# gtonkinhill/tracs

Hardware: AMD Instinct MI355X
Metric: sample-pairs/sec for 10kx5Mbp SNP+transcluster distance (higher is better)
Workload: dtype u32; 1 GPU; 10000 samples x 5000000 sites, consensus (ACGTN) alignment, mu = 0.0001 per sample + 0.01 N (SURVEY 8d): pairsnp (d + compared sites) + transcluster (P, E(K)), all 49995000 pairs; samples=10000, sites=5000000, pairs=49995000, encoding=consensus, kernel=mfma, distinct_keys=174015, partition=one rank: no exchange, workload_name=sparse, streams=1, checksum_d=49010657734

## Files before the change

tracs_amd/csrc/site_lists.hip:

```cpp
#include "pairsnp_kernels.h"

#include <algorithm>
#include <cstdio>
#include <cstddef>
#include <cstdlib>

namespace tracs {

struct SiteLists {
    uint4 *lines = nullptr;
    unsigned long long n_lines = 0;
    unsigned long long *p_off = nullptr;
    unsigned *p_ent = nullptr;
    uint4 *qlines = nullptr;
    unsigned long long n_qlines = 0;
    unsigned qw = 32;
    unsigned long long *s_off = nullptr;
    unsigned *s_ent = nullptr;
    unsigned *c_p = nullptr;
    uint4 *T = nullptr;
    size_t tgroups = 0;
    unsigned short *slots = nullptr;
    size_t batches = 0;
    uint4 *nnl_mask = nullptr;
    uint4 *lst_mask = nullptr;
    unsigned *off_lst = nullptr;
    size_t sites = 0, groups = 0;
    unsigned long long tot_p = 0, tot_nnl = 0;
    unsigned max_row = 0;
    unsigned max_row_pad = 0;
    unsigned long long slot_lines = 0;
    unsigned rows[4] = {0, 0, 0, 0};
    int n_rows = 0;
    unsigned *ns = nullptr;
    size_t ns_words = 0;
    unsigned *site_of = nullptr;
};
constexpr int ENT_SHIFT = 5;
constexpr unsigned ENT_HOLE = 0xFFFFFFFFu;
constexpr unsigned ENT_LONG = 0x80000000u;

__device__ __forceinline__ unsigned word_of(const uint4 &v, int w) { return w == 0 ? v.x : w == 1 ? v.y : w == 2 ? v.z : v.w; }

__device__ __forceinline__ unsigned lst_rank(const uint4 &m, unsigned off_g, int w, int b)
{
    unsigned r = off_g;
    if (w > 0) r += __popc(m.x);
    if (w > 1) r += __popc(m.y);
    if (w > 2) r += __popc(m.z);
    return r + __popc(word_of(m, w) & ((1u << b) - 1u));
}

__device__ __forceinline__ bool row_wanted(const MinorBuild &mb, size_t s)
{
    if (mb.n_rows == 0) return true;
    return (s >= mb.rows[0] && s < mb.rows[1]) || (mb.n_rows > 1 && s >= mb.rows[2] && s < mb.rows[3]);
}

#ifndef TRACS_PL_THREADS
#define TRACS_PL_THREADS 512
#endif
constexpr unsigned PL_THREADS = TRACS_PL_THREADS, PL_MIN = 1024, PL_CAP = 8192, PL_CHUNK = 4096, PL_PER_THREAD = PL_CHUNK / PL_THREADS;
static_assert(PL_PER_THREAD * PL_THREADS == PL_CHUNK && PL_PER_THREAD <= 32 && 64 % PL_PER_THREAD == 0, "p_lists_kernel: a thread's samples sit in one flag word");
__device__ __forceinline__ bool p_lists_in_lds(unsigned group_entries) { return group_entries >= PL_MIN && group_entries <= PL_CAP; }
constexpr unsigned SITE_THREADS = 128;

struct N8Encoder {
    uint4 *lines;
    unsigned line, next_ovf, fill, prev;
    unsigned left;
    unsigned a0, a1, a2, a3;
    static constexpr unsigned DONE = 0xFFFFu;
    __device__ __forceinline__ void put(unsigned b, bool more)
    {
        a0 = __builtin_amdgcn_alignbit(a1, a0, 8); a1 = __builtin_amdgcn_alignbit(a2, a1, 8); a2 = __builtin_amdgcn_alignbit(a3, a2, 8);
        a3 = (a3 >> 8) | (b << 24);
        fill++;
        const bool full = fill == N8_PAYLOAD;
        if ((fill & 15u) == 0u || full) {
            const unsigned nx = more ? next_ovf : N8_NONE;
            lines[(size_t)line * 8 + (full ? 7u : (fill >> 4) - 1u)] = full ? make_uint4(a1, a2, a3, nx) : make_uint4(a0, a1, a2, a3);
            if (full) {
                if (more) { line = next_ovf++; fill = 0; }
                else fill = DONE;
            }
        }
    }
    __device__ __forceinline__ void finish()
    {
        if (fill == DONE) return;
        const uint4 ones = make_uint4(0xFFFFFFFFu, 0xFFFFFFFFu, 0xFFFFFFFFu, 0xFFFFFFFFu);
        while ((fill & 15u) != 0u && fill != DONE) put(0xFFu, false);
        if (fill == DONE) return;
        for (unsigned q = fill >> 4; q < 8u; q++) lines[(size_t)line * 8 + q] = ones;
    }
};

#ifndef TRACS_SITE_WAVES
#define TRACS_SITE_WAVES 8
#endif
#if TRACS_SITE_WAVES > 0
#define TRACS_SITE_ATTR __attribute__((amdgpu_waves_per_eu(TRACS_SITE_WAVES, TRACS_SITE_WAVES)))
#else
#define TRACS_SITE_ATTR
#endif
template <unsigned PIECE_SAMPLES>
__global__ __launch_bounds__(SITE_THREADS) TRACS_SITE_ATTR void site_lists_kernel(const MinorBuild mb, size_t n_pad, unsigned n,
                                                         unsigned long long *__restrict__ p_off, unsigned *__restrict__ p_ent,
                                                         unsigned *__restrict__ qd, uint2 *__restrict__ E, unsigned *__restrict__ e_cnt,
                                                         uint4 *__restrict__ lines,
                                                         unsigned *__restrict__ c_p)
{
    constexpr unsigned PIECE_WORDS = PIECE_SAMPLES / 32, BM_STRIDE = PIECE_WORDS + 1;
    __shared__ unsigned bm[SITES_PER_GROUP * BM_STRIDE];
    __shared__ unsigned kp[SITES_PER_GROUP], ovf[SITES_PER_GROUP], curP[SITES_PER_GROUP], rk[SITES_PER_GROUP];
    __shared__ unsigned qb[SITES_PER_GROUP];
    unsigned *const curQ = ovf;
    __shared__ unsigned long long bP[SITES_PER_GROUP];
    __shared__ unsigned short queue[PIECE_SAMPLES];
    __shared__ unsigned qn[2];
    const size_t g = blockIdx.x;
    const int tid = threadIdx.x;
    const unsigned lane = tid & 63u, wave = tid >> 6;
    if (g == 0 && tid == 0) p_off[mb.sites] = mb.tot_p;
    const uint4 m4 = mb.lst_mask[g], q4 = mb.minor_mask[g];
    if ((m4.x | m4.y | m4.z | m4.w) == 0u) return;
    const unsigned m[4] = {m4.x, m4.y, m4.z, m4.w};
    const unsigned mp[4] = {q4.x, q4.y, q4.z, q4.w};
    const bool any_minor = (q4.x | q4.y | q4.z | q4.w) != 0u;
    const bool from_planes = any_minor && !p_lists_in_lds(mb.gP[g]);
    if (from_planes && tid == 0) e_cnt[g] = 0xFFFFFFFFu;
    static_assert(SITE_THREADS == SITES_PER_GROUP, "thread = site");
    const int tw = tid >> 5, tb = tid & 31;
    const bool mine = (m[tw] >> tb) & 1u;
    const bool want_n = mb.gram == 0;
    const unsigned my_cn = (mine && want_n) ? mb.cntN[g * SITES_PER_GROUP + tid] : 0u;
    {
        const unsigned c = my_cn;
        kp[tid] = (mine && ((mp[tw] >> tb) & 1u)) ? mb.cntP[g * SITES_PER_GROUP + tid] : 0u;
        ovf[tid] = mine ? n8_lines_max(c, n) - 1u : 0u;
        curP[tid] = 0;
        if (tid < 2) qn[tid] = 0;
    }
    __syncthreads();
    const Transpose32 transpose(lane);
    N8Encoder enc{lines, 0u, 0u, 0u, 0xFFFFFFFFu, 0u, 0u, 0u, 0u, 0u};
    if (mine) {
        unsigned long long pp = 0;
        unsigned po = 0, pq = 0;
        for (int t = 0; t < tid; t++) { pp += kp[t]; po += ovf[t]; pq += kp[t] / 31u; }
        const unsigned rank = lst_rank(m4, mb.off_lst[g], tw, tb);
        bP[tid] = mb.baseP[g] + pp; rk[tid] = rank;
        qb[tid] = (unsigned)(mb.sites + mb.baseQ[g] + pq);
        p_off[rank] = bP[tid];
        enc.line = rank;
        enc.left = my_cn;
        enc.next_ovf = (unsigned)(mb.sites + mb.baseO[g] + po);
    }
    __syncthreads();
    curQ[tid] = 0;
    const uint4 RX = mb.ref_x[g], RY = mb.ref_y[g];
    const uint4 *base = mb.planes + (g * NPLANES) * n_pad;
    const uint4 zero4 = make_uint4(0u, 0u, 0u, 0u);
    auto place = [&](unsigned s, unsigned st, unsigned code) {
        const unsigned slot = (code & 16u) ? atomicAdd(&curP[st], 1u) : kp[st] - 1u - atomicAdd(&curQ[st], 1u);
        const unsigned long long pos = bP[st] + slot;
        const bool is_long = kp[st] > P_SHORT_MAX;
        if (is_long) {
            const unsigned qs = slot + 1u, qt = qs / (mb.qw - 1u);
            qd[(size_t)(qt ? qb[st] + qt - 1u : rk[st]) * mb.qw + (qs - qt * (mb.qw - 1u))] = (s << ENT_SHIFT) | code;
        } else {
            p_ent[pos] = (s << ENT_SHIFT) | code;
        }
        E[pos] = (code & 16u) ? make_uint2(s, (is_long ? ENT_LONG : 0u) | (rk[st] << ENT_SHIFT) | code) : make_uint2(ENT_HOLE, 0u);
    };
    for (unsigned piece = 0; piece < n; piece += PIECE_SAMPLES) {
        const unsigned par = (piece / PIECE_SAMPLES) & 1u;
        unsigned sl = wave;
        uint4 N_next = zero4;
        unsigned long long fl_next = 0ull;
        {
            const unsigned s = piece + sl * 64u + lane;
            if (s < n) { if (want_n) N_next = base[4 * n_pad + s]; if (from_planes) fl_next = mb.flags[g * mb.flag_words + (s >> 6)]; }
        }
        for (; sl < PIECE_SAMPLES / 64u; sl += SITE_THREADS / 64u) {
            const unsigned s = piece + sl * 64u + lane;
            const uint4 N = N_next;
            const unsigned long long fl = fl_next;
            {
                const unsigned sn = s + SITE_THREADS;
                N_next = zero4; fl_next = 0ull;
                if (sl + SITE_THREADS / 64u < PIECE_SAMPLES / 64u && sn < n) { if (want_n) N_next = base[4 * n_pad + sn]; if (from_planes) fl_next = mb.flags[g * mb.flag_words + (sn >> 6)]; }
            }
            if (!want_n) {
            } else if (piece + sl * 64u < n) {
                const unsigned col = sl * 2u + (lane >> 5), r = lane & 31u;
                bm[(0u + r) * BM_STRIDE + col] = transpose(N.x & m[0]);
                bm[(32u + r) * BM_STRIDE + col] = transpose(N.y & m[1]);
                bm[(64u + r) * BM_STRIDE + col] = transpose(N.z & m[2]);
                bm[(96u + r) * BM_STRIDE + col] = transpose(N.w & m[3]);
            } else {
                const unsigned col = sl * 2u + (lane >> 5), r = lane & 31u;
                bm[(0u + r) * BM_STRIDE + col] = 0u; bm[(32u + r) * BM_STRIDE + col] = 0u;
                bm[(64u + r) * BM_STRIDE + col] = 0u; bm[(96u + r) * BM_STRIDE + col] = 0u;
            }
            const bool flagged = s < n && ((fl >> (s & 63u)) & 1ull);
            const unsigned long long fm = __ballot(flagged);
            if (fm) {
                unsigned qb = 0;
                if (lane == 0) qb = atomicAdd(&qn[par], (unsigned)__popcll(fm));
                qb = __shfl(qb, 0, 64);
                if (flagged) queue[qb + __builtin_amdgcn_mbcnt_hi((unsigned)(fm >> 32), __builtin_amdgcn_mbcnt_lo((unsigned)fm, 0u))] = (unsigned short)(s - piece);
            }
        }
        __syncthreads();
        const unsigned qcount = qn[par];
        if (tid == 0) qn[par ^ 1u] = 0;
        for (unsigned k = tid; k < qcount; k += SITE_THREADS) {
            const unsigned s = piece + queue[k];
            const uint4 A = base[s], C = base[n_pad + s], G = base[2 * n_pad + s], T = base[3 * n_pad + s];
            unsigned listed_w = 0;
#pragma unroll
            for (int w = 0; w < 4; w++) {
                const unsigned a = word_of(A, w), c = word_of(C, w), gg = word_of(G, w), t = word_of(T, w), isn = a & c & gg & t;
                const unsigned rx = word_of(RX, w), ry = word_of(RY, w);
                const unsigned ra = ~rx & ~ry, rc = rx & ~ry, rg = ~rx & ry, rt = rx & ry;
                const unsigned has_ref = (a & ra) | (c & rc) | (gg & rg) | (t & rt);
                const unsigned only_ref = ~((a ^ ra) | (c ^ rc) | (gg ^ rg) | (t ^ rt));
                unsigned pm = (a | c | gg | t) & ~isn & ~only_ref & mp[w];
                while (pm) {
                    const int b = __ffs(pm) - 1;
                    pm &= pm - 1;
                    const unsigned mask = ((a >> b) & 1u) | (((c >> b) & 1u) << 1) | (((gg >> b) & 1u) << 2) | (((t >> b) & 1u) << 3);
                    const unsigned code = (((has_ref >> b) & 1u) ? 0u : 16u) | mask;
                    place(s, (unsigned)(w * 32 + b), code);
                    listed_w += code >> 4;
                }
            }
            if (listed_w) atomicAdd(&c_p[s], listed_w);
        }
        if (mine && my_cn != 0u) {
            static_assert(PIECE_WORDS <= 64, "one bit per word of the piece");
            const unsigned *rowp = bm + (unsigned)tid * BM_STRIDE;
            unsigned long long nz = 0;
#pragma unroll
            for (unsigned c = 0; c < PIECE_WORDS; c++) nz |= (unsigned long long)(rowp[c] != 0u ? 1u : 0u) << c;
            unsigned w = 0, c = 0, gap = 0;
            bool have = false;
            for (;;) {
                if (!have) {
                    if (w == 0u) {
                        if (nz == 0ull) break;
                        c = __ffsll((long long)nz) - 1; nz &= nz - 1;
                        w = rowp[c];
                    }
                    const unsigned b = __ffs(w) - 1;
                    w &= w - 1;
                    const unsigned smp = piece + 32u * c + b;
                    gap = smp - enc.prev;
                    enc.prev = smp; enc.left--;
                    have = true;
                }
                const bool skip = gap >= N8_SKIP;
                enc.put(skip ? N8_SKIP : gap, skip || enc.left != 0u);
                if (skip) gap -= N8_SKIP; else have = false;
            }
        }
        __syncthreads();
    }
    if (mine) {
        if (want_n) enc.finish();
        if (from_planes && kp[tid] > P_SHORT_MAX) { qd[(size_t)rk[tid] * mb.qw] = kp[tid] | (curP[tid] << 16); qd[(size_t)rk[tid] * mb.qw + mb.qw - 1u] = qb[tid]; }
    }
}

__global__ __launch_bounds__(PL_THREADS) void p_lists_kernel(const MinorBuild mb, size_t n_pad, unsigned n, unsigned *__restrict__ p_ent,
                                                             unsigned *__restrict__ qd, uint2 *__restrict__ E, unsigned *__restrict__ e_cnt,
                                                             int holes, unsigned *__restrict__ c_p)
{
    __shared__ unsigned sorted[PL_CAP];
    __shared__ unsigned w1off[SITES_PER_GROUP];
    __shared__ unsigned char site_of[PL_CAP];
    __shared__ unsigned kp[SITES_PER_GROUP], loff[SITES_PER_GROUP], curP[SITES_PER_GROUP], curQ[SITES_PER_GROUP], rk[SITES_PER_GROUP], qb[SITES_PER_GROUP];
    __shared__ unsigned short queue[PL_CHUNK];
    __shared__ unsigned wtot[PL_THREADS / 64];
    const size_t g = blockIdx.x;
    const unsigned tid = threadIdx.x, lane = tid & 63u, wave = tid >> 6;
    const uint4 q4 = mb.minor_mask[g];
    if ((q4.x | q4.y | q4.z | q4.w) == 0u) return;
    const unsigned long long baseP = mb.baseP[g];
    if (!p_lists_in_lds(mb.gP[g])) return;
    if (tid < SITES_PER_GROUP) {
        const bool mine = (word_of(q4, (int)(tid >> 5)) >> (tid & 31u)) & 1u;
        kp[tid] = mine ? mb.cntP[g * SITES_PER_GROUP + tid] : 0u;
        curP[tid] = 0; curQ[tid] = 0;
    }
    __syncthreads();
    if (tid < SITES_PER_GROUP) {
        unsigned pp = 0, pq = 0;
        for (unsigned t = 0; t < tid; t++) { pp += kp[t]; pq += kp[t] / 31u; }
        loff[tid] = pp;
        rk[tid] = lst_rank(mb.lst_mask[g], mb.off_lst[g], (int)(tid >> 5), (int)(tid & 31u));
        qb[tid] = (unsigned)(mb.sites + mb.baseQ[g] + pq);
    }
    const uint4 RX = mb.ref_x[g], RY = mb.ref_y[g];
    const uint4 *base = mb.planes + (g * NPLANES) * n_pad;
    const unsigned mp[4] = {q4.x, q4.y, q4.z, q4.w};
#if defined(TRACS_PL_CUT) && TRACS_PL_CUT == 3
    for (unsigned c0 = 0; c0 < 0; c0 += PL_CHUNK) {
#else
    for (unsigned c0 = 0; c0 < n; c0 += PL_CHUNK) {
#endif
        const unsigned s0 = c0 + PL_PER_THREAD * tid;
        unsigned bits = s0 < n ? (unsigned)(mb.flags[g * mb.flag_words + (s0 >> 6)] >> (s0 & 63u)) & ((1u << PL_PER_THREAD) - 1u) : 0u;
        const unsigned cnt = (unsigned)__popc(bits);
        unsigned x = cnt;
#pragma unroll
        for (int off = 1; off < 64; off <<= 1) { const unsigned o = __shfl_up(x, off, 64); if ((int)lane >= off) x += o; }
        if (lane == 63u) wtot[wave] = x;
        __syncthreads();
        unsigned pos = x - cnt, qcount = 0;
#pragma unroll
        for (unsigned w = 0; w < PL_THREADS / 64u; w++) { const unsigned t = wtot[w]; if (w < wave) pos += t; qcount += t; }
        while (bits) { const unsigned b = (unsigned)__ffs(bits) - 1u; bits &= bits - 1u; queue[pos++] = (unsigned short)(PL_PER_THREAD * tid + b); }
        __syncthreads();
        for (unsigned k0 = 0; k0 < qcount; k0 += 2u * PL_THREADS) {
            const unsigned ka = k0 + tid, kb = k0 + PL_THREADS + tid;
            const bool ha = ka < qcount, hb = kb < qcount;
            const unsigned sa = c0 + (ha ? queue[ka] : 0u), sb = c0 + (hb ? queue[kb] : 0u);
            const uint4 z = make_uint4(0u, 0u, 0u, 0u);
            const uint4 Aa = ha ? base[sa] : z, Ca = ha ? base[n_pad + sa] : z, Ga = ha ? base[2 * n_pad + sa] : z, Ta = ha ? base[3 * n_pad + sa] : z;
            const uint4 Ab = hb ? base[sb] : z, Cb = hb ? base[n_pad + sb] : z, Gb = hb ? base[2 * n_pad + sb] : z, Tb = hb ? base[3 * n_pad + sb] : z;
            auto sample = [&](unsigned s, const uint4 &A, const uint4 &C, const uint4 &G, const uint4 &T) {
                unsigned listed_w = 0;
#pragma unroll
                for (int w = 0; w < 4; w++) {
                    const unsigned a = word_of(A, w), c = word_of(C, w), gg = word_of(G, w), t = word_of(T, w), isn = a & c & gg & t;
                    const unsigned rx = word_of(RX, w), ry = word_of(RY, w);
                    const unsigned ra = ~rx & ~ry, rc = rx & ~ry, rg = ~rx & ry, rt = rx & ry;
                    const unsigned has_ref = (a & ra) | (c & rc) | (gg & rg) | (t & rt);
                    const unsigned only_ref = ~((a ^ ra) | (c ^ rc) | (gg ^ rg) | (t ^ rt));
                    unsigned pm = (a | c | gg | t) & ~isn & ~only_ref & mp[w];
                    while (pm) {
                        const unsigned b = (unsigned)__ffs(pm) - 1u;
                        pm &= pm - 1u;
                        const unsigned mask = ((a >> b) & 1u) | (((c >> b) & 1u) << 1) | (((gg >> b) & 1u) << 2) | (((t >> b) & 1u) << 3);
                        const unsigned code = (((has_ref >> b) & 1u) ? 0u : 16u) | mask;
                        const unsigned st = (unsigned)w * 32u + b;
                        const unsigned slot = (code & 16u) ? atomicAdd(&curP[st], 1u) : kp[st] - 1u - atomicAdd(&curQ[st], 1u);
                        sorted[loff[st] + slot] = (s << ENT_SHIFT) | code;
                        site_of[loff[st] + slot] = (unsigned char)st;
                        listed_w += code >> 4;
                    }
                }
#ifndef TRACS_PL_NO_CP
                if (listed_w) atomicAdd(&c_p[s], listed_w);
#endif
            };
#if defined(TRACS_PL_CUT) && TRACS_PL_CUT == 2
            if ((Aa.x ^ Ca.y ^ Ga.z ^ Ta.w ^ Ab.x ^ Cb.y ^ Gb.z ^ Tb.w) == 0x12345679u) c_p[0] = 1u;
#else
            if (ha) sample(sa, Aa, Ca, Ga, Ta);
            if (hb) sample(sb, Ab, Cb, Gb, Tb);
#endif
        }
    }
#if defined(TRACS_PL_CUT) && (TRACS_PL_CUT == 1 || TRACS_PL_CUT == 2)
    return;
#endif
    __syncthreads();
    if (tid < 64u) {
        const unsigned a = curP[tid], b = curP[64 + tid];
        unsigned xa = a, xb = b;
#pragma unroll
        for (int off = 1; off < 64; off <<= 1) {
            const unsigned oa = __shfl_up(xa, off, 64), ob = __shfl_up(xb, off, 64);
            if ((int)tid >= off) { xa += oa; xb += ob; }
        }
        const unsigned ta = __shfl(xa, 63, 64), tb = __shfl(xb, 63, 64);
        w1off[tid] = xa - a; w1off[64 + tid] = ta + xb - b;
        if (tid == 0) e_cnt[g] = holes ? 0xFFFFFFFFu : ta + tb;
    }
    __syncthreads();
    const unsigned total = mb.gP[g];
    for (unsigned i = tid; i < total; i += PL_THREADS) {
        const unsigned ent = sorted[i], st = site_of[i];
        const bool is_long = kp[st] > P_SHORT_MAX;
        const uint2 ev = make_uint2(ent >> ENT_SHIFT, (is_long ? ENT_LONG : 0u) | (rk[st] << ENT_SHIFT) | (ent & 31u));
        if (holes) E[baseP + i] = (ent & 16u) ? ev : make_uint2(ENT_HOLE, 0u);
        else if (ent & 16u) E[baseP + w1off[st] + (i - loff[st])] = ev;
        if (!is_long) p_ent[baseP + i] = ent;
    }
    const unsigned qw = mb.qw, per = qw - 1u;
    const unsigned hw = tid / qw, l = tid % qw;
    for (unsigned st = hw; st < SITES_PER_GROUP; st += PL_THREADS / qw) {
        const unsigned k = kp[st];
        if (k <= P_SHORT_MAX) continue;
        const unsigned lo = loff[st], lines_n = k / per + 1u;
        for (unsigned j = 0; j < lines_n; j++) {
            const unsigned qs = per * j + l;
            unsigned v = 0u;
            if (l == per) v = j == 0u ? qb[st] : 0u;
            else if (qs == 0u) v = k | (curP[st] << 16);
            else if (qs <= k) v = sorted[lo + qs - 1u];
            qd[(size_t)(j ? qb[st] + j - 1u : rk[st]) * qw + l] = v;
        }
    }
}

__global__ __launch_bounds__(256) void listed_entries_kernel(const uint2 *__restrict__ E, unsigned long long count,
                                                             const unsigned long long *__restrict__ off, unsigned *__restrict__ cur,
                                                             unsigned *__restrict__ ent)
{
    const unsigned long long k = (unsigned long long)blockIdx.x * 256 + threadIdx.x;
    if (k >= count) return;
    const uint2 e = E[k];
    if (e.x == ENT_HOLE) return;
    ent[off[e.x] + atomicAdd(&cur[e.x], 1u)] = e.y;
}

constexpr unsigned ENT_TILE_THREADS = 1024, ENT_PER_THREAD = 8, ENT_TILE = ENT_TILE_THREADS * ENT_PER_THREAD;
constexpr unsigned ENT_GROUPS = 64;
__global__ __launch_bounds__(ENT_TILE_THREADS) void entries_to_buckets_kernel(const uint2 *__restrict__ E, const unsigned *__restrict__ e_cnt,
                                                                              const unsigned *__restrict__ gP, const unsigned long long *__restrict__ baseP,
// ... 660 lines not shown
                    const unsigned y = wi * 32u + b;
                    if (c && y >= c0 && y < c1) atomicAdd(&row[y - c0], 0u - c);
                }
#pragma unroll
                for (int jx = 0; jx < 8; jx++) pl[jx] = 0;
                since = 0;
            };
            if (active) {
                const unsigned *col = ns + wi;
                unsigned long long e = e0 + grp;
                for (; e + 7ull * ngrp < e1; e += 8ull * ngrp) {
                    unsigned xs[8];
#pragma unroll
                    for (int k = 0; k < 8; k++) {
                        const unsigned ent = s_ent[e + (unsigned long long)k * ngrp];
                        xs[k] = __builtin_nontemporal_load(col + (size_t)site_of[(ent & ~ENT_LONG) >> ENT_SHIFT] * ns_words);
                    }
                    sliced_add8(pl, xs);
                    if (++since == 31u) flush();
                }
                for (; e < e1; e += ngrp) {
                    const unsigned ent = s_ent[e];
                    sliced_add(pl, __builtin_nontemporal_load(col + (size_t)site_of[(ent & ~ENT_LONG) >> ENT_SHIFT] * ns_words));
                    if (++since >= 24u) flush();
                }
                if (since) flush();
            }
        }
    } else if constexpr (!GRAM) {
        Walk<CLAMP> W;
        W.init(lines, row + chunk + 64 + wave * (WALK_LDS_PER_WAVE / 4), lane);
        W.neg4lo = 0u - 4u * c0; W.dump4 = 4u * (span + lane); W.val = 0xFFFFFFFFu; W.cut = 0u;
        for (unsigned long long base = e0 + (unsigned long long)wave * 64; base < e1; base += (unsigned long long)nwaves * 64) {
            const unsigned long long e = base + lane;
            const unsigned ent = e < e1 ? s_ent[e] : 0u;
            W.drain_lines_to(31);
            W.push_line(e < e1, (ent & ~ENT_LONG) >> ENT_SHIFT);
        }
        W.finish();
    }
    __syncthreads();
    if (upper) {
        const unsigned cx = c_p[x];
        for (unsigned j = up0 + threadIdx.x; j < up1; j += blockDim.x) {
            const unsigned t = row[j - c0] + cx + c_p[j];
            if (t) dist[(size_t)x * ld + j] += t;
        }
    }
    if (lower) {
        unsigned *dst = S + (size_t)(x - row_begin) * s_pitch;
        for (unsigned y = lw0 + threadIdx.x; y < lw1; y += blockDim.x) dst[y - row_begin] = row[y - c0];
    }
}

__global__ __launch_bounds__(256) void transpose_add_kernel(const unsigned *__restrict__ S, size_t s_pitch, unsigned n, unsigned row_begin,
                                                            unsigned row_end, unsigned col_begin, unsigned *__restrict__ dist, size_t ld)
{
    __shared__ unsigned tile[32][33];
    const unsigned xb = row_begin + blockIdx.x * 32, yb = row_begin + blockIdx.y * 32;
    if (xb + 31 <= yb) return;
    const unsigned tx = threadIdx.x & 31, ty = threadIdx.x >> 5;
#pragma unroll
    for (int k = 0; k < 4; k++) {
        const unsigned x = xb + ty + 8 * k, y = yb + tx;
        tile[ty + 8 * k][tx] = (x < n && y < row_end && y < x) ? S[(size_t)(x - row_begin) * s_pitch + (y - row_begin)] : 0u;
    }
    __syncthreads();
#pragma unroll
    for (int k = 0; k < 4; k++) {
        const unsigned y = yb + ty + 8 * k, x = xb + tx;
        const unsigned v = tile[tx][ty + 8 * k];
        if (v && x < n && y < row_end && y < x && x >= col_begin) dist[(size_t)y * ld + x] += v;
    }
}

__global__ __launch_bounds__(256) void site_of_rank_kernel(const uint4 *__restrict__ mask, const unsigned *__restrict__ off, size_t groups,
                                                           unsigned *__restrict__ site_of)
{
    const size_t g = (size_t)blockIdx.x * 256 + threadIdx.x;
    if (g >= groups) return;
    const uint4 m4 = mask[g];
    const unsigned m[4] = {m4.x, m4.y, m4.z, m4.w};
    unsigned o = off[g];
#pragma unroll
    for (int w = 0; w < 4; w++) {
        unsigned xw = m[w];
        while (xw) { const unsigned b = __ffs(xw) - 1; site_of[o++] = (unsigned)(g * SITES_PER_GROUP + w * 32 + b); xw &= xw - 1; }
    }
}

void minority_lists_free(tracs_alignment *a)
{
    if (!a) return;
    if (a->lists) pack_stage_count_gone(&a->lists->slot_lines);
    delete a->lists;
    a->lists = nullptr;
}

int minority_lists_build(tracs_alignment *a, const MinorBuild &mb_, hipStream_t stream, int *ok)
{
    *ok = 0;
    minority_lists_free(a);
    MinorBuild mb = mb_;
    const size_t n = a->n, L = mb.sites, groups = a->groups;
    if (L == 0 || L >= (1ull << 26) || n >= (1ull << 27)) return TRACS_OK;
    auto *g = new SiteLists();
    auto fail_soft = [&]() { (void)hipGetLastError(); pack_stage_count_gone(&g->slot_lines); delete g; return TRACS_OK; };
#define SL_TRY(x) do { if ((x) != hipSuccess) return fail_soft(); } while (0)
    g->sites = L; g->groups = groups; g->tot_p = mb.tot_p; g->tot_nnl = mb.tot_nnl;
    g->n_rows = mb.n_rows;
    for (int k = 0; k < 4; k++) g->rows[k] = mb.rows[k];
    g->n_lines = mb.gram ? 0ull : (unsigned long long)L + mb.tot_o;
    g->tgroups = (groups + 15) / 16 * 16;
    SL_TRY(pack_alloc(a, (g->n_lines + 1) * 128, reinterpret_cast<void **>(&g->lines)));
    SL_TRY(pack_alloc(a, (L + 1) * 8, reinterpret_cast<void **>(&g->p_off)));
    SL_TRY(pack_alloc(a, std::max<size_t>(mb.tot_p, 1) * 4, reinterpret_cast<void **>(&g->p_ent)));
    g->n_qlines = mb.long_p ? (unsigned long long)L + mb.tot_q : 0ull;
    g->qw = mb.qw;
    SL_TRY(pack_alloc(a, (g->n_qlines + 1) * (size_t)g->qw * 4, reinterpret_cast<void **>(&g->qlines)));
    SL_TRY(pack_alloc(a, (n + 1) * 8, reinterpret_cast<void **>(&g->s_off)));
    SL_TRY(pack_alloc(a, std::max<size_t>(mb.tot_p, 1) * 4, reinterpret_cast<void **>(&g->s_ent)));
    SL_TRY(pack_alloc(a, std::max<size_t>(n, 1) * 4, reinterpret_cast<void **>(&g->c_p)));
    SL_TRY(pack_alloc(a, groups * sizeof(uint4), reinterpret_cast<void **>(&g->lst_mask)));
    SL_TRY(pack_alloc(a, groups * sizeof(unsigned), reinterpret_cast<void **>(&g->off_lst)));
    const bool bitmaps = mb.tot_nnl > 0;
    static const int env_slots = [] { const char *e = getenv("TRACS_ROW_LISTS"); return e ? atoi(e) : -1; }();
    g->batches = (g->tgroups + SLOT_GROUPS - 1) / SLOT_GROUPS;
    const bool row_slots = bitmaps && (env_slots >= 0 ? env_slots != 0 : (double)mb.tot_nnl <= SLOT_MEAN_MAX * (double)n * (double)g->batches);
    if (row_slots) {
        SL_TRY(pack_alloc(a, n * g->batches * SLOT_BYTES, reinterpret_cast<void **>(&g->slots)));
        SL_TRY(pack_alloc(a, groups * sizeof(uint4), reinterpret_cast<void **>(&g->nnl_mask)));
    } else if (bitmaps) SL_TRY(pack_alloc(a, n * g->tgroups * sizeof(uint4), reinterpret_cast<void **>(&g->T)));
    unsigned *cnt = nullptr, *e_cnt = nullptr;
    uint2 *E = nullptr, *tmp = nullptr;
    int rc;
    if ((rc = workspace_get(60, (2 * std::max<size_t>(n, 1) + 8 + 256) * 4, reinterpret_cast<void **>(&cnt))) ||
        (rc = workspace_get(61, std::max<size_t>(groups, 1) * sizeof(unsigned), reinterpret_cast<void **>(&e_cnt))) ||
        (rc = workspace_get(62, std::max<size_t>(mb.tot_p, 1) * sizeof(uint2), reinterpret_cast<void **>(&E)))) { delete g; return rc; }
    unsigned *cur = cnt + std::max<size_t>(n, 1), *d_max = cur + std::max<size_t>(n, 1), *bcur = d_max + 8;
    unsigned shift = 0;
    while (n && ((n - 1) >> shift) >= 256u) shift++;
    const bool two_pass = mb.tot_p >= ENT_TILE && mb.tot_p < (1ull << 32) && shift <= 10 &&
                          workspace_get(63, (size_t)mb.tot_p * sizeof(uint2), reinterpret_cast<void **>(&tmp)) == TRACS_OK;
    if (!two_pass) { (void)hipGetLastError(); set_error(""); }
    SL_TRY(hipMemsetAsync(cnt, 0, (2 * std::max<size_t>(n, 1) + 8 + 256) * 4, stream));
    SL_TRY(hipMemsetAsync(g->c_p, 0, std::max<size_t>(n, 1) * 4, stream));
    SL_TRY(hipMemcpyAsync(g->lst_mask, mb.lst_mask, groups * sizeof(uint4), hipMemcpyDeviceToDevice, stream));
    SL_TRY(hipMemcpyAsync(g->off_lst, mb.off_lst, groups * sizeof(unsigned), hipMemcpyDeviceToDevice, stream));
    if (row_slots) SL_TRY(hipMemcpyAsync(g->nnl_mask, mb.nnl_mask, groups * sizeof(uint4), hipMemcpyDeviceToDevice, stream));
    const double plane_b = (double)groups * (double)a->n_pad * sizeof(uint4);
#ifndef TRACS_SITE_PIECE
#define TRACS_SITE_PIECE 512
#endif
    hipLaunchKernelGGL((site_lists_kernel<TRACS_SITE_PIECE>), dim3((unsigned)groups), dim3(SITE_THREADS), 0, stream, mb, a->n_pad, (unsigned)n, g->p_off, g->p_ent, reinterpret_cast<unsigned *>(g->qlines), E, e_cnt, g->lines, g->c_p);
    if (mb.max_gp >= PL_MIN)
        hipLaunchKernelGGL(p_lists_kernel, dim3((unsigned)groups), dim3(PL_THREADS), 0, stream, mb, a->n_pad, (unsigned)n, g->p_ent, reinterpret_cast<unsigned *>(g->qlines), E, e_cnt, two_pass ? 0 : 1, g->c_p);
    const double flagged = (double)std::min<unsigned long long>(mb.tot_p, (unsigned long long)n * groups);
    pack_stage_mark("lists: per site", stream, (mb.gram ? 0.0 : plane_b) + (double)groups * SITES_PER_GROUP * 8.0 + std::min(flagged * 4.0 * 128.0, 4.0 * plane_b),
                    (mb.gram ? 0.0 : (double)L * 128.0 * 2.0) + (double)mb.tot_p * 12.0 + (double)L * 8.0 + (double)(mb.tot_q + std::min<unsigned long long>(L, mb.tot_p)) * 8.0);
    hipLaunchKernelGGL(scan_counts_kernel, dim3(1), dim3(1024), 0, stream, g->c_p, n, g->s_off);
    if (mb.tot_p) {
        if (two_pass) {
            const unsigned buckets = (unsigned)(((n - 1) >> shift) + 1);
            hipLaunchKernelGGL(entries_to_buckets_kernel, dim3((unsigned)((groups + ENT_GROUPS - 1) / ENT_GROUPS)), dim3(ENT_TILE_THREADS), 0, stream, E, e_cnt, mb.gP, mb.baseP,
                               groups, shift, (unsigned)n, g->s_off, bcur, tmp);
            const unsigned per_bucket = (unsigned)std::min<unsigned long long>(64, std::max<unsigned long long>(1, mb.tot_p / buckets / ENT_TILE + 1));
            hipLaunchKernelGGL(buckets_to_samples_kernel, dim3(per_bucket, buckets), dim3(ENT_TILE_THREADS), 0, stream, tmp, shift, (unsigned)n, g->s_off, cur, g->s_ent);
        } else {
            hipLaunchKernelGGL(listed_entries_kernel, dim3((unsigned)((mb.tot_p + 255) / 256)), dim3(256), 0, stream, E, mb.tot_p, g->s_off, cur, g->s_ent);
        }
    }
    pack_stage_mark("listed entries per sample", stream, (double)std::min<unsigned long long>(mb.tot_p, 2 * L) * (two_pass ? 16.0 : 8.0) + (double)n * 4.0,
                    (double)std::min<unsigned long long>(mb.tot_p, 2 * L) * (two_pass ? 12.0 : 4.0) + (double)n * 12.0);
    if (row_slots) {
        unsigned long long *d_lines = reinterpret_cast<unsigned long long *>(d_max + 2);
        const unsigned chunks = (unsigned)std::min<size_t>(64, std::max<size_t>(1, g->batches / 2));
        const size_t bpc = (g->batches + chunks - 1) / chunks;
        const dim3 grid((unsigned)((n + 31) / 32), (unsigned)((g->batches + bpc - 1) / bpc));
        hipLaunchKernelGGL(row_slots_kernel, grid, dim3(256), 0, stream, mb, a->n_pad, (unsigned)n, groups, g->batches, bpc, g->slots, a->c_counted, d_lines);
        hipLaunchKernelGGL(max_count_kernel, dim3((unsigned)((n + 255) / 256)), dim3(256), 0, stream, a->c_counted, n, d_max);
        pack_stage_mark("N slots of the rows", stream, plane_b, 0.0);
        pack_stage_written_later(&g->slot_lines, 128.0);
        static_assert(offsetof(SiteLists, slot_lines) == offsetof(SiteLists, max_row) + 8, "max_row and slot_lines come back in one copy");
        SL_TRY(hipMemcpyAsync(&g->max_row, d_max, 16, hipMemcpyDeviceToHost, stream));
    } else if (bitmaps) {
        const size_t octs = g->tgroups / NB_GW;
        const unsigned chunks = (unsigned)std::min<size_t>(64, std::max<size_t>(1, octs / 16));
        const size_t opc = (octs + chunks - 1) / chunks;
        const dim3 grid((unsigned)((n + 4 * NB_SW - 1) / (4 * NB_SW)), (unsigned)((octs + opc - 1) / opc));
        hipLaunchKernelGGL(n_bitmap_kernel, grid, dim3(256), 0, stream, mb, a->n_pad, (unsigned)n, groups, g->tgroups, opc, g->T, a->c_counted);
        hipLaunchKernelGGL(max_count_kernel, dim3((unsigned)((n + 255) / 256)), dim3(256), 0, stream, a->c_counted, n, d_max);
        double rows = (double)n;
        if (mb.n_rows) { rows = 0.0; for (int k = 0; k < mb.n_rows; k++) rows += (double)(std::min<size_t>(mb.rows[2 * k + 1], n) - std::min<size_t>(mb.rows[2 * k], n)); }
        pack_stage_mark("N bitmaps of the rows", stream, plane_b, rows * (double)g->tgroups * sizeof(uint4));
        SL_TRY(hipMemcpyAsync(&g->max_row, d_max, 4, hipMemcpyDeviceToHost, stream));
    }
    if (mb.gram == 2) {
        g->ns_words = ns_words_for(a->n_pad);
        SL_TRY(pack_alloc(a, groups * 128 * g->ns_words * 4, reinterpret_cast<void **>(&g->ns)));
        SL_TRY(pack_alloc(a, std::max<size_t>(L, 1) * 4, reinterpret_cast<void **>(&g->site_of)));
        launch_ns_build(a->planes, a->n_pad, (unsigned)groups, g->ns, g->ns_words, stream);
        hipLaunchKernelGGL(site_of_rank_kernel, dim3((unsigned)((groups + 255) / 256)), dim3(256), 0, stream, g->lst_mask, g->off_lst, groups, g->site_of);
        pack_stage_mark("N plane site-major (NS)", stream, plane_b, (double)groups * 128.0 * (double)g->ns_words * 4.0);
    }
    SL_TRY(hipGetLastError());
#undef SL_TRY
    a->lists = g;
    *ok = 1;
    return TRACS_OK;
}

constexpr unsigned ROW_CHUNK_MAX = 36800;
static unsigned row_chunk(size_t n) { return (unsigned)std::min<size_t>((n + 63) / 64 * 64, ROW_CHUNK_MAX); }
static constexpr size_t kWalkLds = (size_t)(TRACS_NN_THREADS / 64) * WALK_LDS_PER_WAVE;

int nn_rows_add(tracs_alignment *a, size_t row_begin, size_t row_end, size_t col_begin, unsigned *ncomp, size_t ld, int add_terms,
                unsigned lu, hipStream_t stream)
{
    const SiteLists *g = a->lists;
    if (!g || (!g->T && !g->slots)) { set_error("nn_rows_add: lists not built"); return TRACS_E_ARG; }
    const size_t n = a->n;
    const unsigned chunk = row_chunk(n);
    const size_t lds = (size_t)chunk * 4 + 256 + kWalkLds;
    int dev = 0;
    (void)hipGetDevice(&dev);
    static bool attr_set[64] = {false};
    if (dev >= 0 && dev < 64 && !attr_set[dev]) {
        const void *fns[4] = {reinterpret_cast<const void *>(nn_rows_kernel<true, false>), reinterpret_cast<const void *>(nn_rows_kernel<false, false>),
                              reinterpret_cast<const void *>(nn_rows_kernel<true, true>), reinterpret_cast<const void *>(nn_rows_kernel<false, true>)};
        for (const void *fn : fns) TRACS_HIP_CHECK(hipFuncSetAttribute(fn, hipFuncAttributeMaxDynamicSharedMemorySize, (int)ROW_CHUNK_MAX * 4 + 256 + (int)kWalkLds));
        attr_set[dev] = true;
    }
    const unsigned target = (unsigned)std::min<unsigned long long>(1u << 30, std::max<unsigned long long>(8192ull, g->tot_nnl / 2048ull));
    const char *seg_env = getenv("TRACS_NN_SEGMENT_MB");
    const unsigned long long seg_bytes = (seg_env ? strtoull(seg_env, nullptr, 10) : 256ull) << 20;
    const unsigned segments = seg_bytes ? (unsigned)std::min<unsigned long long>(NN_MAX_SPLITS, std::max<unsigned long long>(1, (g->n_lines * 128ull + seg_bytes - 1) / seg_bytes)) : 1u;
    const unsigned splits = (unsigned)std::min<unsigned long long>(NN_MAX_SPLITS, std::max<unsigned long long>(segments, ((unsigned long long)g->max_row + target - 1) / target));
    const dim3 grid((unsigned)(row_end - row_begin), (unsigned)((n + chunk - 1) / chunk), splits);
    const uint4 *nplane = a->planes + 4 * a->n_pad;
#define TRACS_NN_LAUNCH(CL, SL) hipLaunchKernelGGL((nn_rows_kernel<CL, SL>), grid, dim3(TRACS_NN_THREADS), lds, stream, g->T, g->tgroups, \
        reinterpret_cast<const unsigned *>(g->slots), nplane, a->n_pad, g->nnl_mask, g->lst_mask, g->off_lst, g->groups, g->lines, \
        a->c_counted, (unsigned)n, (unsigned)row_begin, (unsigned)col_begin, chunk, target, segments, ncomp, ld, add_terms, lu)
    if (grid.y == 1) {
        if (g->slots) TRACS_NN_LAUNCH(false, true); else TRACS_NN_LAUNCH(false, false);
    } else {
        if (g->slots) TRACS_NN_LAUNCH(true, true); else TRACS_NN_LAUNCH(true, false);
    }
#undef TRACS_NN_LAUNCH
    TRACS_HIP_CHECK(hipGetLastError());
    return TRACS_OK;
}

int minority_fixup(tracs_alignment *a, size_t row_begin, size_t row_end, size_t col_begin, unsigned *dist, size_t ld, hipStream_t stream)
{
    const SiteLists *g = a->lists;
    if (!g || g->tot_p == 0) return TRACS_OK;
    const size_t n = a->n;
    const unsigned chunk = row_chunk(n);
    const size_t lds = (size_t)chunk * 4 + 256 + (size_t)16 * WALK_LDS_PER_WAVE;
    int dev = 0;
    (void)hipGetDevice(&dev);
    static bool attr_set[64] = {false};
    if (dev >= 0 && dev < 64 && !attr_set[dev]) {
        const int fix_lds = (int)ROW_CHUNK_MAX * 4 + 256 + 16 * (int)WALK_LDS_PER_WAVE;
        const void *fns[12] = {reinterpret_cast<const void *>(minor_fixup_kernel<true, 32, false>), reinterpret_cast<const void *>(minor_fixup_kernel<false, 32, false>),
                               reinterpret_cast<const void *>(minor_fixup_kernel<true, 64, false>), reinterpret_cast<const void *>(minor_fixup_kernel<false, 64, false>),
                               reinterpret_cast<const void *>(minor_fixup_kernel<true, 32, true>), reinterpret_cast<const void *>(minor_fixup_kernel<false, 32, true>),
                               reinterpret_cast<const void *>(minor_fixup_kernel<true, 64, true>), reinterpret_cast<const void *>(minor_fixup_kernel<false, 64, true>),
                               reinterpret_cast<const void *>(minor_fixup_kernel<true, 32, false, true>), reinterpret_cast<const void *>(minor_fixup_kernel<false, 32, false, true>),
                               reinterpret_cast<const void *>(minor_fixup_kernel<true, 64, false, true>), reinterpret_cast<const void *>(minor_fixup_kernel<false, 64, false, true>)};
        for (const void *fn : fns) TRACS_HIP_CHECK(hipFuncSetAttribute(fn, hipFuncAttributeMaxDynamicSharedMemorySize, fix_lds));
        attr_set[dev] = true;
    }
    const size_t s_pitch = (row_end - row_begin + 63) / 64 * 64;
    unsigned *S = nullptr;
    const int rc = workspace_get(46, (n - row_begin) * s_pitch * sizeof(unsigned), reinterpret_cast<void **>(&S));
    if (rc) return rc;
    const dim3 grid((unsigned)(n - row_begin), (unsigned)((n + chunk - 1) / chunk));
#define TRACS_FIXUP_LAUNCH(CL, QWV) hipLaunchKernelGGL((minor_fixup_kernel<CL, QWV, GR, NR>), grid, dim3(1024), lds, stream, g->s_off, g->s_ent, g->p_off, g->p_ent, \
        reinterpret_cast<const unsigned *>(g->qlines), g->lines, g->c_p, (unsigned)n, (unsigned)row_begin, (unsigned)row_end, (unsigned)col_begin, chunk, dist, ld, S, s_pitch, \
        g->ns, g->ns_words, g->site_of)
    if (a->nw_rows) {
        constexpr bool GR = false, NR = true;
        if (grid.y == 1) { if (g->qw == 64u) TRACS_FIXUP_LAUNCH(false, 64); else TRACS_FIXUP_LAUNCH(false, 32); }
        else { if (g->qw == 64u) TRACS_FIXUP_LAUNCH(true, 64); else TRACS_FIXUP_LAUNCH(true, 32); }
    } else if (a->nw_gram) {
        constexpr bool GR = true, NR = false;
        if (grid.y == 1) { if (g->qw == 64u) TRACS_FIXUP_LAUNCH(false, 64); else TRACS_FIXUP_LAUNCH(false, 32); }
        else { if (g->qw == 64u) TRACS_FIXUP_LAUNCH(true, 64); else TRACS_FIXUP_LAUNCH(true, 32); }
    } else {
        constexpr bool GR = false, NR = false;
        if (grid.y == 1) { if (g->qw == 64u) TRACS_FIXUP_LAUNCH(false, 64); else TRACS_FIXUP_LAUNCH(false, 32); }
        else { if (g->qw == 64u) TRACS_FIXUP_LAUNCH(true, 64); else TRACS_FIXUP_LAUNCH(true, 32); }
    }
#undef TRACS_FIXUP_LAUNCH
    const dim3 tgrid((unsigned)((n - row_begin + 31) / 32), (unsigned)((row_end - row_begin + 31) / 32));
    hipLaunchKernelGGL(transpose_add_kernel, tgrid, dim3(256), 0, stream, S, s_pitch, (unsigned)n, (unsigned)row_begin, (unsigned)row_end,
                       (unsigned)col_begin, dist, ld);
    TRACS_HIP_CHECK(hipGetLastError());
    return TRACS_OK;
}

}

extern "C" {

size_t tracs_debug_lists(const tracs_alignment *a, int what, void *out, size_t cap)
{
    using namespace tracs;
    if (!a || !a->lists || !out) return 0;
    const SiteLists *g = a->lists;
    const void *src = nullptr;
// ... 51 lines not shown
```

Baseline: 2.312 billion pairs/s.

## Stage N8 encoder lines in an LDS image and write whole lines out

Adds an IMG variant of the per-site list kernel. Each site's 128-byte N8 output line is built in a padded LDS image and written to global memory as full 128-byte lines when the line fills or at kernel end, replacing byte-wise global puts plus a padding pass. It also prefetches the whole next piece's N-plane and flag words into registers while the listed-entry loop runs. The cost is more LDS and registers per block, with occupancy hints dropped to 4 waves per EU. It is on by default unless the TRACS_N8_IMAGE environment variable disables it.

```diff
diff --git a/tracs_amd/csrc/site_lists.hip b/tracs_amd/csrc/site_lists.hip
--- a/tracs_amd/csrc/site_lists.hip
+++ b/tracs_amd/csrc/site_lists.hip
@@ -99,12 +99,17 @@
 #ifndef TRACS_SITE_WAVES
 #define TRACS_SITE_WAVES 8
 #endif
+constexpr unsigned N8_IMG_STRIDE = 132, N8_IMG_DWORDS = N8_IMG_STRIDE / 4;
+static_assert(N8_IMG_STRIDE % 4 == 0 && N8_IMG_STRIDE % 128 != 0 && N8_IMG_STRIDE >= N8_PAYLOAD + 4, "image: a padded 128-byte line");
+#ifndef TRACS_SITE_IMAGE_WAVES
+#define TRACS_SITE_IMAGE_WAVES 4
+#endif
 #if TRACS_SITE_WAVES > 0
-#define TRACS_SITE_ATTR __attribute__((amdgpu_waves_per_eu(TRACS_SITE_WAVES, TRACS_SITE_WAVES)))
+#define TRACS_SITE_ATTR __attribute__((amdgpu_waves_per_eu(IMG ? TRACS_SITE_IMAGE_WAVES : TRACS_SITE_WAVES, IMG ? TRACS_SITE_IMAGE_WAVES : TRACS_SITE_WAVES)))
 #else
 #define TRACS_SITE_ATTR
 #endif
-template <unsigned PIECE_SAMPLES>
+template <unsigned PIECE_SAMPLES, bool IMG>
 __global__ __launch_bounds__(SITE_THREADS) TRACS_SITE_ATTR void site_lists_kernel(const MinorBuild mb, size_t n_pad, unsigned n,
                                                          unsigned long long *__restrict__ p_off, unsigned *__restrict__ p_ent,
                                                          unsigned *__restrict__ qd, uint2 *__restrict__ E, unsigned *__restrict__ e_cnt,
@@ -112,7 +117,15 @@
                                                          unsigned *__restrict__ c_p)
 {
     constexpr unsigned PIECE_WORDS = PIECE_SAMPLES / 32, BM_STRIDE = PIECE_WORDS + 1;
+    constexpr unsigned SLABS = PIECE_SAMPLES / 64u / (SITE_THREADS / 64u);
+    static_assert(SLABS * 64u * (SITE_THREADS / 64u) == PIECE_SAMPLES, "a piece: whole slabs for every wave");
     __shared__ unsigned bm[SITES_PER_GROUP * BM_STRIDE];
+    unsigned *img = nullptr, *cur_line = nullptr;
+    if constexpr (IMG) {
+        __shared__ unsigned img_s[SITES_PER_GROUP * N8_IMG_DWORDS];
+        __shared__ unsigned cur_line_s[SITES_PER_GROUP];
+        img = img_s; cur_line = cur_line_s;
+    }
     __shared__ unsigned kp[SITES_PER_GROUP], ovf[SITES_PER_GROUP], curP[SITES_PER_GROUP], rk[SITES_PER_GROUP];
     __shared__ unsigned qb[SITES_PER_GROUP];
     unsigned *const curQ = ovf;
@@ -156,6 +169,10 @@
         enc.line = rank;
         enc.left = my_cn;
         enc.next_ovf = (unsigned)(mb.sites + mb.baseO[g] + po);
+        if constexpr (IMG) {
+#pragma unroll
+            for (unsigned k = 0; k < N8_IMG_DWORDS; k++) img[(unsigned)tid * N8_IMG_DWORDS + k] = N8_NONE;
+        }
     }
     __syncthreads();
     curQ[tid] = 0;
@@ -174,74 +191,110 @@
         }
         E[pos] = (code & 16u) ? make_uint2(s, (is_long ? ENT_LONG : 0u) | (rk[st] << ENT_SHIFT) | code) : make_uint2(ENT_HOLE, 0u);
     };
+    auto slab = [&](unsigned piece, unsigned par, unsigned sl, const uint4 &N, unsigned long long fl) {
+        const unsigned s = piece + sl * 64u + lane;
+        if (!want_n) {
+        } else if (piece + sl * 64u < n) {
+            const unsigned col = sl * 2u + (lane >> 5), r = lane & 31u;
+            bm[(0u + r) * BM_STRIDE + col] = transpose(N.x & m[0]);
+            bm[(32u + r) * BM_STRIDE + col] = transpose(N.y & m[1]);
+            bm[(64u + r) * BM_STRIDE + col] = transpose(N.z & m[2]);
+            bm[(96u + r) * BM_STRIDE + col] = transpose(N.w & m[3]);
+        } else {
+            const unsigned col = sl * 2u + (lane >> 5), r = lane & 31u;
+            bm[(0u + r) * BM_STRIDE + col] = 0u; bm[(32u + r) * BM_STRIDE + col] = 0u;
+            bm[(64u + r) * BM_STRIDE + col] = 0u; bm[(96u + r) * BM_STRIDE + col] = 0u;
+        }
+        const bool flagged = s < n && ((fl >> (s & 63u)) & 1ull);
+        const unsigned long long fm = __ballot(flagged);
+        if (fm) {
+            unsigned qb = 0;
+            if (lane == 0) qb = atomicAdd(&qn[par], (unsigned)__popcll(fm));
+            qb = __shfl(qb, 0, 64);
+            if (flagged) queue[qb + __builtin_amdgcn_mbcnt_hi((unsigned)(fm >> 32), __builtin_amdgcn_mbcnt_lo((unsigned)fm, 0u))] = (unsigned short)(s - piece);
+        }
+    };
+    auto listed = [&](unsigned s, const uint4 &A, const uint4 &C, const uint4 &G, const uint4 &T) {
+        unsigned listed_w = 0;
+#pragma unroll
+        for (int w = 0; w < 4; w++) {
+            const unsigned a = word_of(A, w), c = word_of(C, w), gg = word_of(G, w), t = word_of(T, w), isn = a & c & gg & t;
+            const unsigned rx = word_of(RX, w), ry = word_of(RY, w);
+            const unsigned ra = ~rx & ~ry, rc = rx & ~ry, rg = ~rx & ry, rt = rx & ry;
+            const unsigned has_ref = (a & ra) | (c & rc) | (gg & rg) | (t & rt);
+            const unsigned only_ref = ~((a ^ ra) | (c ^ rc) | (gg ^ rg) | (t ^ rt));
+            unsigned pm = (a | c | gg | t) & ~isn & ~only_ref & mp[w];
+            while (pm) {
+                const int b = __ffs(pm) - 1;
+                pm &= pm - 1;
+                const unsigned mask = ((a >> b) & 1u) | (((c >> b) & 1u) << 1) | (((gg >> b) & 1u) << 2) | (((t >> b) & 1u) << 3);
+                const unsigned code = (((has_ref >> b) & 1u) ? 0u : 16u) | mask;
+                place(s, (unsigned)(w * 32 + b), code);
+                listed_w += code >> 4;
+            }
+        }
+        if (listed_w) atomicAdd(&c_p[s], listed_w);
+    };
+    uint4 Nq[SLABS];
+    unsigned long long flq[SLABS];
+    [[maybe_unused]] auto fetch = [&](unsigned piece) {
+#pragma unroll
+        for (unsigned k = 0; k < SLABS; k++) {
+            const unsigned s = piece + (wave + k * (SITE_THREADS / 64u)) * 64u + lane;
+            Nq[k] = zero4; flq[k] = 0ull;
+            if (s < n) { if (want_n) Nq[k] = base[4 * n_pad + s]; if (from_planes) flq[k] = mb.flags[g * mb.flag_words + (s >> 6)]; }
+        }
+    };
+    if constexpr (IMG) fetch(0u);
     for (unsigned piece = 0; piece < n; piece += PIECE_SAMPLES) {
         const unsigned par = (piece / PIECE_SAMPLES) & 1u;
-        unsigned sl = wave;
-        uint4 N_next = zero4;
-        unsigned long long fl_next = 0ull;
-        {
-            const unsigned s = piece + sl * 64u + lane;
-            if (s < n) { if (want_n) N_next = base[4 * n_pad + s]; if (from_planes) fl_next = mb.flags[g * mb.flag_words + (s >> 6)]; }
-        }
-        for (; sl < PIECE_SAMPLES / 64u; sl += SITE_THREADS / 64u) {
-            const unsigned s = piece + sl * 64u + lane;
-            const uint4 N = N_next;
-            const unsigned long long fl = fl_next;
+        if constexpr (IMG) {
+#pragma unroll
+            for (unsigned k = 0; k < SLABS; k++) slab(piece, par, wave + k * (SITE_THREADS / 64u), Nq[k], flq[k]);
+        } else {
+            unsigned sl = wave;
+            uint4 N_next = zero4;
+            unsigned long long fl_next = 0ull;
             {
-                const unsigned sn = s + SITE_THREADS;
-                N_next = zero4; fl_next = 0ull;
-                if (sl + SITE_THREADS / 64u < PIECE_SAMPLES / 64u && sn < n) { if (want_n) N_next = base[4 * n_pad + sn]; if (from_planes) fl_next = mb.flags[g * mb.flag_words + (sn >> 6)]; }
+                const unsigned s = piece + sl * 64u + lane;
+                if (s < n) { if (want_n) N_next = base[4 * n_pad + s]; if (from_planes) fl_next = mb.flags[g * mb.flag_words + (s >> 6)]; }
             }
-            if (!want_n) {
-            } else if (piece + sl * 64u < n) {
-                const unsigned col = sl * 2u + (lane >> 5), r = lane & 31u;
-                bm[(0u + r) * BM_STRIDE + col] = transpose(N.x & m[0]);
-                bm[(32u + r) * BM_STRIDE + col] = transpose(N.y & m[1]);
-                bm[(64u + r) * BM_STRIDE + col] = transpose(N.z & m[2]);
-                bm[(96u + r) * BM_STRIDE + col] = transpose(N.w & m[3]);
-            } else {
-                const unsigned col = sl * 2u + (lane >> 5), r = lane & 31u;
-                bm[(0u + r) * BM_STRIDE + col] = 0u; bm[(32u + r) * BM_STRIDE + col] = 0u;
-                bm[(64u + r) * BM_STRIDE + col] = 0u; bm[(96u + r) * BM_STRIDE + col] = 0u;
-            }
-            const bool flagged = s < n && ((fl >> (s & 63u)) & 1ull);
-            const unsigned long long fm = __ballot(flagged);
-            if (fm) {
-                unsigned qb = 0;
-                if (lane == 0) qb = atomicAdd(&qn[par], (unsigned)__popcll(fm));
-                qb = __shfl(qb, 0, 64);
-                if (flagged) queue[qb + __builtin_amdgcn_mbcnt_hi((unsigned)(fm >> 32), __builtin_amdgcn_mbcnt_lo((unsigned)fm, 0u))] = (unsigned short)(s - piece);
+            for (; sl < PIECE_SAMPLES / 64u; sl += SITE_THREADS / 64u) {
+                const unsigned s = piece + sl * 64u + lane;
+                const uint4 N = N_next;
+                const unsigned long long fl = fl_next;
+                {
+                    const unsigned sn = s + SITE_THREADS;
+                    N_next = zero4; fl_next = 0ull;
+                    if (sl + SITE_THREADS / 64u < PIECE_SAMPLES / 64u && sn < n) { if (want_n) N_next = base[4 * n_pad + sn]; if (from_planes) fl_next = mb.flags[g * mb.flag_words + (sn >> 6)]; }
+                }
+                slab(piece, par, sl, N, fl);
             }
         }
         __syncthreads();
         const unsigned qcount = qn[par];
         if (tid == 0) qn[par ^ 1u] = 0;
-        for (unsigned k = tid; k < qcount; k += SITE_THREADS) {
-            const unsigned s = piece + queue[k];
-            const uint4 A = base[s], C = base[n_pad + s], G = base[2 * n_pad + s], T = base[3 * n_pad + s];
-            unsigned listed_w = 0;
-#pragma unroll
-            for (int w = 0; w < 4; w++) {
-                const unsigned a = word_of(A, w), c = word_of(C, w), gg = word_of(G, w), t = word_of(T, w), isn = a & c & gg & t;
-                const unsigned rx = word_of(RX, w), ry = word_of(RY, w);
-                const unsigned ra = ~rx & ~ry, rc = rx & ~ry, rg = ~rx & ry, rt = rx & ry;
-                const unsigned has_ref = (a & ra) | (c & rc) | (gg & rg) | (t & rt);
-                const unsigned only_ref = ~((a ^ ra) | (c ^ rc) | (gg ^ rg) | (t ^ rt));
-                unsigned pm = (a | c | gg | t) & ~isn & ~only_ref & mp[w];
-                while (pm) {
-                    const int b = __ffs(pm) - 1;
-                    pm &= pm - 1;
-                    const unsigned mask = ((a >> b) & 1u) | (((c >> b) & 1u) << 1) | (((gg >> b) & 1u) << 2) | (((t >> b) & 1u) << 3);
-                    const unsigned code = (((has_ref >> b) & 1u) ? 0u : 16u) | mask;
-                    place(s, (unsigned)(w * 32 + b), code);
-                    listed_w += code >> 4;
-                }
+        if constexpr (IMG) {
+            const bool h0 = (unsigned)tid < qcount;
+            const unsigned s0 = piece + (h0 ? queue[tid] : 0u);
+            uint4 A0 = make_uint4(0u, 0u, 0u, 0u), C0 = A0, G0 = A0, T0 = A0;
+            if (h0) { A0 = base[s0]; C0 = base[n_pad + s0]; G0 = base[2 * n_pad + s0]; T0 = base[3 * n_pad + s0]; }
+            if (piece + PIECE_SAMPLES < n) fetch(piece + PIECE_SAMPLES);
+            if (h0) listed(s0, A0, C0, G0, T0);
+            for (unsigned k = tid + SITE_THREADS; k < qcount; k += SITE_THREADS) {
+                const unsigned s = piece + queue[k];
+                listed(s, base[s], base[n_pad + s], base[2 * n_pad + s], base[3 * n_pad + s]);
             }
-            if (listed_w) atomicAdd(&c_p[s], listed_w);
+        } else {
+            for (unsigned k = tid; k < qcount; k += SITE_THREADS) {
+                const unsigned s = piece + queue[k];
+                listed(s, base[s], base[n_pad + s], base[2 * n_pad + s], base[3 * n_pad + s]);
+            }
         }
         if (mine && my_cn != 0u) {
             static_assert(PIECE_WORDS <= 64, "one bit per word of the piece");
             const unsigned *rowp = bm + (unsigned)tid * BM_STRIDE;
+            [[maybe_unused]] unsigned *const my_img = img + (unsigned)tid * N8_IMG_DWORDS;
             unsigned long long nz = 0;
 #pragma unroll
             for (unsigned c = 0; c < PIECE_WORDS; c++) nz |= (unsigned long long)(rowp[c] != 0u ? 1u : 0u) << c;
@@ -262,14 +315,39 @@
                     have = true;
                 }
                 const bool skip = gap >= N8_SKIP;
-                enc.put(skip ? N8_SKIP : gap, skip || enc.left != 0u);
+                if constexpr (IMG) {
+                    reinterpret_cast<unsigned char *>(my_img)[enc.fill] = (unsigned char)(skip ? N8_SKIP : gap);
+                    enc.fill++;
+                    if (enc.fill == N8_PAYLOAD && (skip || enc.left != 0u)) {
+                        my_img[N8_PAYLOAD / 4u] = enc.next_ovf;
+                        uint4 *dst = lines + (size_t)enc.line * 8;
+#pragma unroll
+                        for (unsigned q = 0; q < 8u; q++) dst[q] = make_uint4(my_img[4u * q], my_img[4u * q + 1u], my_img[4u * q + 2u], my_img[4u * q + 3u]);
+#pragma unroll
+                        for (unsigned q = 0; q < 32u; q++) my_img[q] = N8_NONE;
+                        enc.line = enc.next_ovf++; enc.fill = 0;
+                    }
+                } else {
+                    enc.put(skip ? N8_SKIP : gap, skip || enc.left != 0u);
+                }
                 if (skip) gap -= N8_SKIP; else have = false;
             }
         }
         __syncthreads();
     }
+    if constexpr (IMG) {
+        cur_line[tid] = mine ? enc.line : N8_NONE;
+        __syncthreads();
+#pragma unroll
+        for (unsigned it = 0; it < 8u; it++) {
+            const unsigned st = it * (SITE_THREADS / 8u) + ((unsigned)tid >> 3), q = (unsigned)tid & 7u;
+            const unsigned ln = cur_line[st];
+            const unsigned *src = img + st * N8_IMG_DWORDS + 4u * q;
+            if (ln != N8_NONE) lines[(size_t)ln * 8 + q] = make_uint4(src[0], src[1], src[2], src[3]);
+        }
+    }
     if (mine) {
-        if (want_n) enc.finish();
+        if constexpr (!IMG) { if (want_n) enc.finish(); }
         if (from_planes && kp[tid] > P_SHORT_MAX) { qd[(size_t)rk[tid] * mb.qw] = kp[tid] | (curP[tid] << 16); qd[(size_t)rk[tid] * mb.qw + mb.qw - 1u] = qb[tid]; }
     }
 }
@@ -1236,12 +1314,17 @@
 #ifndef TRACS_SITE_PIECE
 #define TRACS_SITE_PIECE 512
 #endif
-    hipLaunchKernelGGL((site_lists_kernel<TRACS_SITE_PIECE>), dim3((unsigned)groups), dim3(SITE_THREADS), 0, stream, mb, a->n_pad, (unsigned)n, g->p_off, g->p_ent, reinterpret_cast<unsigned *>(g->qlines), E, e_cnt, g->lines, g->c_p);
+    static const bool env_image = [] { const char *e = getenv("TRACS_N8_IMAGE"); return !e || atoi(e) != 0; }();
+    const bool image = env_image && !mb.gram;
+    if (image)
+        hipLaunchKernelGGL((site_lists_kernel<TRACS_SITE_PIECE, true>), dim3((unsigned)groups), dim3(SITE_THREADS), 0, stream, mb, a->n_pad, (unsigned)n, g->p_off, g->p_ent, reinterpret_cast<unsigned *>(g->qlines), E, e_cnt, g->lines, g->c_p);
+    else
+        hipLaunchKernelGGL((site_lists_kernel<TRACS_SITE_PIECE, false>), dim3((unsigned)groups), dim3(SITE_THREADS), 0, stream, mb, a->n_pad, (unsigned)n, g->p_off, g->p_ent, reinterpret_cast<unsigned *>(g->qlines), E, e_cnt, g->lines, g->c_p);
     if (mb.max_gp >= PL_MIN)
         hipLaunchKernelGGL(p_lists_kernel, dim3((unsigned)groups), dim3(PL_THREADS), 0, stream, mb, a->n_pad, (unsigned)n, g->p_ent, reinterpret_cast<unsigned *>(g->qlines), E, e_cnt, two_pass ? 0 : 1, g->c_p);
     const double flagged = (double)std::min<unsigned long long>(mb.tot_p, (unsigned long long)n * groups);
     pack_stage_mark("lists: per site", stream, (mb.gram ? 0.0 : plane_b) + (double)groups * SITES_PER_GROUP * 8.0 + std::min(flagged * 4.0 * 128.0, 4.0 * plane_b),
-                    (mb.gram ? 0.0 : (double)L * 128.0 * 2.0) + (double)mb.tot_p * 12.0 + (double)L * 8.0 + (double)(mb.tot_q + std::min<unsigned long long>(L, mb.tot_p)) * 8.0);
+                    (mb.gram ? 0.0 : (double)L * 128.0 * (image ? 1.0 : 2.0)) + (double)mb.tot_p * 12.0 + (double)L * 8.0 + (double)(mb.tot_q + std::min<unsigned long long>(L, mb.tot_p)) * 8.0);
     hipLaunchKernelGGL(scan_counts_kernel, dim3(1), dim3(1024), 0, stream, g->c_p, n, g->s_off);
     if (mb.tot_p) {
         if (two_pass) {
```

Result: slower. 2.189 billion pairs/s (-5.3%).
